# OpenSpaceAI/Nesie

Hardware: AMD Instinct MI355X
Metric: ScanNet scenes/sec (fwd+bwd, 40k pts, bs=8) (higher is better)
Workload: dtype f32; 1 GPU; Nesie-VoteNet supervised pretrain step (nesie-votenet-scannet-pretrain-10%): fwd+bwd+AdamW, 40000 pts/scene, fp32, random-init weights; scenes_per_gpu=8, global_batch=8, parallelism=single, world_size=1, hip_graph=True, deterministic_backward=True, index_chain_pipelined=True, forward_cu_budget=232, forward_cu_budget_from_the_head_on=248, grad_allreduce_bytes=10561936, resident_input_scenes=0

## Files before the change

nesie_amd/csrc/interpolate.hip:

```cpp
#include "common.h"
#include <math.h>

namespace nesie {

constexpr int NN_BLOCK = 256;
constexpr int NN_TILE = 1024;

template <int FORM>
__global__ __launch_bounds__(NN_BLOCK) void three_nn_kernel(
    int n, int m, const float *__restrict__ unknown, const float *__restrict__ known,
    float *__restrict__ dist2, int *__restrict__ idx) {
  __shared__ float4 kk[NN_TILE];
  const int bi = blockIdx.y;
  const int q = blockIdx.x * NN_BLOCK + threadIdx.x;
  const bool live = q < n;
  unknown += (size_t)bi * n * 3;
  known += (size_t)bi * m * 3;
  const int qq = live ? q : n - 1;
  const float ux = unknown[qq * 3 + 0], uy = unknown[qq * 3 + 1], uz = unknown[qq * 3 + 2];
  float b1 = INFINITY, b2 = INFINITY, b3 = INFINITY;
  int i1 = 0, i2 = 0, i3 = 0;
  for (int t0 = 0; t0 < m; t0 += NN_TILE) {
    const int tn = m - t0 < NN_TILE ? m - t0 : NN_TILE;
    __syncthreads();
    for (int i = threadIdx.x; i < tn; i += NN_BLOCK)
      kk[i] = make_float4(known[(t0 + i) * 3 + 0], known[(t0 + i) * 3 + 1],
                          known[(t0 + i) * 3 + 2], 0.f);
    __syncthreads();
#pragma unroll 4
    for (int i = 0; i < tn; ++i) {
      const float4 kp = kk[i];
      const float d = sqdist_form<FORM>(ux - kp.x, uy - kp.y, uz - kp.z);
      if (d < b3) {
        const int k = t0 + i;
        if (d < b1) {
          b3 = b2; i3 = i2; b2 = b1; i2 = i1; b1 = d; i1 = k;
        } else if (d < b2) {
          b3 = b2; i3 = i2; b2 = d; i2 = k;
        } else {
          b3 = d; i3 = k;
        }
      }
    }
  }
  if (live) {
    float *od = dist2 + ((size_t)bi * n + q) * 3;
    int *oi = idx + ((size_t)bi * n + q) * 3;
    od[0] = b1; od[1] = b2; od[2] = b3;
    oi[0] = i1; oi[1] = i2; oi[2] = i3;
  }
}

template <int FORM>
__global__ __launch_bounds__(NN_BLOCK) void grid_taps_kernel(
    int kprop, int gp, int m, const float *__restrict__ centre, const float *__restrict__ size,
    const float *__restrict__ heading, const float *__restrict__ mult,
    const float *__restrict__ plane, const float *__restrict__ known, int *__restrict__ idx,
    float *__restrict__ weight, float *__restrict__ rel) {
  __shared__ float4 kk[NN_TILE];
  const int bi = blockIdx.y;
  const int n = kprop * gp;
  const int q = blockIdx.x * NN_BLOCK + threadIdx.x;
  const bool live = q < n;
  const int qq = live ? q : n - 1;
  const int k = qq / gp, g = qq - k * gp;
  const float *c3 = centre + ((size_t)bi * kprop + k) * 3;
  const float *s3 = size + ((size_t)bi * kprop + k) * 3;
  const float cx = c3[0], cy = c3[1], cz = c3[2];
  float l[3];
#pragma unroll
  for (int d = 0; d < 3; ++d) {
    const float f = __fmul_rn(mult[g * 3 + d], s3[d]) / 2.f;
    l[d] = __fadd_rn(f, __fmul_rn(f, plane[g * 3 + d]));
  }
  const float h = heading[(size_t)bi * kprop + k];
  const float ch = cosf(h), sh = sinf(h);
  const float ux = __fadd_rn(__fadd_rn(__fmul_rn(l[0], ch), __fmul_rn(l[1], sh)), cx);
  const float uy = __fadd_rn(__fadd_rn(__fmul_rn(l[0], -sh), __fmul_rn(l[1], ch)), cy);
  const float uz = __fadd_rn(l[2], cz);
  known += (size_t)bi * m * 3;
  float b1 = INFINITY, b2 = INFINITY, b3 = INFINITY;
  int i1 = 0, i2 = 0, i3 = 0;
  for (int t0 = 0; t0 < m; t0 += NN_TILE) {
    const int tn = m - t0 < NN_TILE ? m - t0 : NN_TILE;
    __syncthreads();
    for (int i = threadIdx.x; i < tn; i += NN_BLOCK)
      kk[i] = make_float4(known[(t0 + i) * 3 + 0], known[(t0 + i) * 3 + 1],
                          known[(t0 + i) * 3 + 2], 0.f);
    __syncthreads();
#pragma unroll 4
    for (int i = 0; i < tn; ++i) {
      const float4 kp = kk[i];
      const float d = sqdist_form<FORM>(ux - kp.x, uy - kp.y, uz - kp.z);
      if (d < b3) {
        const int kidx = t0 + i;
        if (d < b1) {
          b3 = b2; i3 = i2; b2 = b1; i2 = i1; b1 = d; i1 = kidx;
        } else if (d < b2) {
          b3 = b2; i3 = i2; b2 = d; i2 = kidx;
        } else {
          b3 = d; i3 = kidx;
        }
      }
    }
  }
  if (live) {
    const size_t o = ((size_t)bi * n + q) * 3;
    const float w1 = 1.f / __fadd_rn(sqrtf(b1), 1e-8f), w2 = 1.f / __fadd_rn(sqrtf(b2), 1e-8f),
                w3 = 1.f / __fadd_rn(sqrtf(b3), 1e-8f);
    const float ws = __fadd_rn(__fadd_rn(w1, w2), w3);
    idx[o] = i1; idx[o + 1] = i2; idx[o + 2] = i3;
    weight[o] = w1 / ws; weight[o + 1] = w2 / ws; weight[o + 2] = w3 / ws;
    rel[o] = ux - cx; rel[o + 1] = uy - cy; rel[o + 2] = uz - cz;
  }
}

constexpr int TI_BLOCK = 256;
constexpr int TI_CH = 8;

__global__ __launch_bounds__(TI_BLOCK) void three_interpolate_kernel(
    int c, int m, int n, const float *__restrict__ points, const int *__restrict__ idx,
    const float *__restrict__ weight, float *__restrict__ out) {
  const int p = blockIdx.x * TI_BLOCK + threadIdx.x;
  const int c0 = blockIdx.y * TI_CH;
  const int bi = blockIdx.z;
  if (p >= n) return;
  const int *ix = idx + ((size_t)bi * n + p) * 3;
  const float *w = weight + ((size_t)bi * n + p) * 3;
  int j0 = ix[0], j1 = ix[1], j2 = ix[2];
  j0 = j0 < 0 ? 0 : (j0 >= m ? m - 1 : j0);
  j1 = j1 < 0 ? 0 : (j1 >= m ? m - 1 : j1);
  j2 = j2 < 0 ? 0 : (j2 >= m ? m - 1 : j2);
  const float w0 = w[0], w1 = w[1], w2 = w[2];
  const int cend = c - c0 < TI_CH ? c - c0 : TI_CH;
#pragma unroll
  for (int i = 0; i < TI_CH; ++i) {
    if (i < cend) {
      const float *src = points + ((size_t)bi * c + c0 + i) * m;
      float r = __fadd_rn(__fadd_rn(__fmul_rn(w0, src[j0]), __fmul_rn(w1, src[j1])),
                          __fmul_rn(w2, src[j2]));
      out[((size_t)bi * c + c0 + i) * n + p] = r;
    }
  }
}

constexpr int TS_Q = 64;

__global__ __launch_bounds__(256) void blend_fwd_kernel(
    int c, int m, int n, int segs, int seg_len, int c_total, int c_offset, int pitch,
    int seg_off, const float *__restrict__ table, const int *__restrict__ idx,
    const float *__restrict__ weight, const float *__restrict__ rel,
    const float *__restrict__ wx, float *__restrict__ out, float *__restrict__ stat_partial,
    int nt, int nb) {
  __shared__ float tile[64][TS_Q + 1];
  __shared__ float red[4][64][2];
  __shared__ int sj[TS_Q][3];
  __shared__ float sw[TS_Q][3];
  __shared__ float sr[TS_Q][3];
  const int bi = blockIdx.x % nb;
  const int q0 = (blockIdx.x / nb) * TS_Q;
  const int per_seg = n / segs;
  const int sg = q0 / per_seg, r0 = q0 - sg * per_seg;
  const int lane = threadIdx.x & 63, wv = threadIdx.x >> 6;
  if (threadIdx.x < TS_Q) {
    const int r = r0 + threadIdx.x;
    const int k = r / seg_len, g = r - k * seg_len;
    const size_t p = (size_t)bi * n + (size_t)(k * segs + sg) * seg_len + g;
#pragma unroll
    for (int t = 0; t < 3; ++t) {
      int j = idx[p * 3 + t];
      sj[threadIdx.x][t] = j < 0 ? 0 : (j >= m ? m - 1 : j);
      sw[threadIdx.x][t] = weight[p * 3 + t];
      sr[threadIdx.x][t] = rel ? rel[p * 3 + t] : 0.f;
    }
  }
  __syncthreads();
  const float *feat = table + (size_t)bi * m * pitch + (size_t)sg * seg_off;
  float *dst = out + (((size_t)bi * segs + sg) * c_total + c_offset) * per_seg + r0;
  for (int c0 = 0; c0 < c; c0 += 64) {
    float x0 = 0.f, x1 = 0.f, x2 = 0.f;
    if (wx) {
      const float *wr = wx + ((size_t)sg * c + c0 + lane) * 3;
      x0 = wr[0]; x1 = wr[1]; x2 = wr[2];
    }
    float a_s = 0.f, a_q = 0.f;
#pragma unroll 4
    for (int i = 0; i < 16; ++i) {
      const int qi = wv * 16 + i;
      const float *f = feat + c0 + lane;
      const float a0 = f[(size_t)sj[qi][0] * pitch], a1 = f[(size_t)sj[qi][1] * pitch],
                  a2 = f[(size_t)sj[qi][2] * pitch];
      float v = __fadd_rn(__fadd_rn(__fmul_rn(sw[qi][0], a0), __fmul_rn(sw[qi][1], a1)),
                          __fmul_rn(sw[qi][2], a2));
      if (wx)
        v = __fadd_rn(__fadd_rn(__fadd_rn(v, __fmul_rn(x0, sr[qi][0])), __fmul_rn(x1, sr[qi][1])),
                      __fmul_rn(x2, sr[qi][2]));
      tile[lane][qi] = v;
      a_s += v; a_q += v * v;
    }
    if (stat_partial) { red[wv][lane][0] = a_s; red[wv][lane][1] = a_q; }
    __syncthreads();
#pragma unroll
    for (int i = 0; i < 4; ++i) {
      const int ch = wv * 16 + i * 4 + (lane >> 4), q4 = (lane & 15) * 4;
      const float4 v = make_float4(tile[ch][q4], tile[ch][q4 + 1], tile[ch][q4 + 2], tile[ch][q4 + 3]);
      float *o = dst + (size_t)(c0 + ch) * per_seg + q4;
      if (nt) st4<true>(o, v); else st4<false>(o, v);
    }
    if (stat_partial && wv == 0) {
      const float ss = (red[0][lane][0] + red[1][lane][0]) + (red[2][lane][0] + red[3][lane][0]);
      const float qq = (red[0][lane][1] + red[1][lane][1]) + (red[2][lane][1] + red[3][lane][1]);
      const int nslice = nb * (per_seg / TS_Q);
      const int slice = bi * (per_seg / TS_Q) + r0 / TS_Q;
      float *pd = stat_partial + ((size_t)(sg * c + c0 + lane) * nslice + slice) * 2;
      pd[0] = ss; pd[1] = qq;
    }
    __syncthreads();
  }
}

__global__ __launch_bounds__(TI_BLOCK) void blend_fwd_generic_kernel(
    int c, int m, int n, int segs, int seg_len, int c_total, int c_offset, int pitch,
    int seg_off, const float *__restrict__ table, const int *__restrict__ idx,
    const float *__restrict__ weight, const float *__restrict__ rel,
    const float *__restrict__ wx, float *__restrict__ out) {
  const int q = blockIdx.x * TI_BLOCK + threadIdx.x;
  const int c0 = blockIdx.y * TI_CH;
  const int bi = blockIdx.z;
  if (q >= n) return;
  const int per_seg = n / segs;
  const int sg = q / per_seg, r = q - sg * per_seg;
  const int k = r / seg_len, g = r - k * seg_len;
  const size_t p = (size_t)bi * n + (size_t)(k * segs + sg) * seg_len + g;
  int j0 = idx[p * 3], j1 = idx[p * 3 + 1], j2 = idx[p * 3 + 2];
  j0 = j0 < 0 ? 0 : (j0 >= m ? m - 1 : j0);
  j1 = j1 < 0 ? 0 : (j1 >= m ? m - 1 : j1);
  j2 = j2 < 0 ? 0 : (j2 >= m ? m - 1 : j2);
  const float w0 = weight[p * 3], w1 = weight[p * 3 + 1], w2 = weight[p * 3 + 2];
  const float rx = rel ? rel[p * 3] : 0.f, ry = rel ? rel[p * 3 + 1] : 0.f,
              rz = rel ? rel[p * 3 + 2] : 0.f;
  const int cend = c - c0 < TI_CH ? c - c0 : TI_CH;
  const float *feat = table + (size_t)bi * m * pitch + (size_t)sg * seg_off + c0;
  float *dst = out + (((size_t)bi * segs + sg) * c_total + c_offset + c0) * per_seg + r;
#pragma unroll
  for (int i = 0; i < TI_CH; ++i) {
    if (i < cend) {
      float v = __fadd_rn(
          __fadd_rn(__fmul_rn(w0, feat[(size_t)j0 * pitch + i]), __fmul_rn(w1, feat[(size_t)j1 * pitch + i])),
          __fmul_rn(w2, feat[(size_t)j2 * pitch + i]));
      if (wx) {
        const float *wr = wx + ((size_t)sg * c + c0 + i) * 3;
        v = __fadd_rn(__fadd_rn(__fadd_rn(v, __fmul_rn(wr[0], rx)), __fmul_rn(wr[1], ry)),
                      __fmul_rn(wr[2], rz));
      }
      dst[(size_t)i * per_seg] = v;
    }
  }
}

constexpr int BL_RUN = 512;

__device__ __forceinline__ unsigned bitonic_sort64(unsigned v, int lane) {
#pragma unroll
  for (int k = 2; k <= 64; k <<= 1) {
#pragma unroll
    for (int j = k >> 1; j >= 1; j >>= 1) {
      const unsigned o = (unsigned)__shfl_xor((int)v, j, 64);
      const bool up = (lane & k) == 0;
      const bool lower = (lane & j) == 0;
      v = (up == lower) ? (v < o ? v : o) : (v > o ? v : o);
    }
  }
  return v;
}

constexpr int BL_SLOTS = 48;

template <int CPT, bool BNB, bool STAGED>
__global__ __launch_bounds__(256, 2) void blend_bwd_rows_kernel(
    int m, int n, int segs, int seg_len, int pitch, int seg_off,
    const float *__restrict__ dy , const int *__restrict__ idx,
    const float *__restrict__ weight, const float *__restrict__ rel,
    float *__restrict__ d_table, float *__restrict__ d_wx_part, int nb, int nruns,
    const float *__restrict__ bnz, const float *__restrict__ bnb,
    float *__restrict__ stage, int *__restrict__ slot_seed) {
  constexpr int C = CPT * 64;
  __shared__ float tile[C * (TS_Q + 1)];
  __shared__ int sj[TS_Q][3];
  __shared__ float sw[TS_Q][3];
  __shared__ float sr[TS_Q][3];
  const int bi = blockIdx.x % nb, run_i = (blockIdx.x / nb) % nruns, sg = blockIdx.x / (nb * nruns);
  const int per_seg = n / segs;
  const int run0 = run_i * BL_RUN;
  const int lane = threadIdx.x & 63, wv = threadIdx.x >> 6;
  const float *src = dy + ((size_t)bi * segs + sg) * C * per_seg;
  const float *zsrc = BNB ? bnz + ((size_t)bi * segs + sg) * C * per_seg : nullptr;
  const int wvu = __builtin_amdgcn_readfirstlane(wv);
  float *dt = d_table + (size_t)bi * m * pitch + (size_t)sg * seg_off + lane;
  float dx[CPT][3];
#pragma unroll
  for (int e = 0; e < CPT; ++e) dx[e][0] = dx[e][1] = dx[e][2] = 0.f;
  const int run_end = run0 + BL_RUN < per_seg ? run0 + BL_RUN : per_seg;
  constexpr int NR = C / 4;
  float traw[NR], zraw[BNB ? NR : 1];
  int pj[3];
  float pw[3], pr[3];
  auto prefetch = [&](int r0) {
    if (threadIdx.x < TS_Q) {
      const int r = r0 + threadIdx.x;
      const int k = r / seg_len, g = r - k * seg_len;
      const size_t p = (size_t)bi * n + (size_t)(k * segs + sg) * seg_len + g;
#pragma unroll
      for (int t = 0; t < 3; ++t) {
        pj[t] = idx[p * 3 + t];
        pw[t] = weight[p * 3 + t];
        pr[t] = rel ? rel[p * 3 + t] : 0.f;
      }
    }
    const unsigned voff = (unsigned)(((size_t)wv * per_seg + lane) * 4);
#pragma unroll
    for (int i = 0; i < NR; ++i) {
      const float *sb_ = src + (size_t)(i * 4) * per_seg + r0;
      traw[i] = *(const float *)((const char *)sb_ + voff);
    }
  };
  auto load_z = [&](int r0) {
    const unsigned voff = (unsigned)(((size_t)wv * per_seg + lane) * 4);
#pragma unroll
    for (int i = 0; i < NR; ++i) {
      const float *zb_ = zsrc + (size_t)(i * 4) * per_seg + r0;
      zraw[i] = *(const float *)((const char *)zb_ + voff);
    }
  };
  auto lds_barrier = [&]() {
    asm volatile("s_waitcnt lgkmcnt(0)" ::: "memory");
    __builtin_amdgcn_s_barrier();
  };
  if (run0 < run_end) prefetch(run0);
  for (int r0 = run0; r0 < run_end; r0 += TS_Q) {
    if (BNB) load_z(r0);
    lds_barrier();
    if (threadIdx.x < TS_Q) {
#pragma unroll
      for (int t = 0; t < 3; ++t) {
        const int j = pj[t];
        sj[threadIdx.x][t] = j < 0 ? 0 : (j >= m ? m - 1 : j);
        sw[threadIdx.x][t] = pw[t];
        sr[threadIdx.x][t] = pr[t];
      }
    }
#pragma unroll
    for (int i = 0; i < NR; ++i) {
      float v = traw[i];
      if (BNB) {
        const float *cf = bnb + ((size_t)sg * C + i * 4 + wvu) * 8;
        const float zz = zraw[i];
        const float gg = __builtin_fmaf(zz, cf[0], cf[1]) > 0.f ? v : 0.f;
        v = __builtin_fmaf(cf[2], gg, __builtin_fmaf(cf[3] - zz, cf[4], cf[5]));
      }
      tile[(i * 4 + wv) * (TS_Q + 1) + lane] = v;
    }
    lds_barrier();
    const int rn = r0 + TS_Q < run_end ? r0 + TS_Q : r0;
    prefetch(rn);
    const int q0 = wv * 16;
    if (d_wx_part) {
#pragma unroll 4
      for (int u = 0; u < 16; ++u) {
        const float r0x = sr[q0 + u][0], r1x = sr[q0 + u][1], r2x = sr[q0 + u][2];
#pragma unroll
        for (int e = 0; e < CPT; ++e) {
          const float v = tile[(e * 64 + lane) * (TS_Q + 1) + q0 + u];
          dx[e][0] += v * r0x; dx[e][1] += v * r1x; dx[e][2] += v * r2x;
        }
      }
    }
    unsigned key = 0xFFFFFFFFu;
    if (lane < 48) key = ((unsigned)sj[q0 + lane / 3][lane % 3] << 6) | (unsigned)lane;
    key = bitonic_sort64(key, lane);
    int cur = -1;
    float acc[CPT];
#pragma unroll
    for (int e = 0; e < CPT; ++e) acc[e] = 0.f;
    const size_t gslot = STAGED ? ((size_t)((size_t)bi * segs + sg) * (per_seg / 16) + (r0 + q0) / 16) * BL_SLOTS : 0;
    int rank = 0;
    if (STAGED) {
      const int sd = lane < 48 ? (int)(key >> 6) : -1;
      const int sp = __shfl_up(sd, 1, 64);
      const bool first = lane < 48 && (lane == 0 || sd != sp);
      const unsigned long long fm = __ballot(first);
      const int nvalid = __popcll(fm);
      if (first) slot_seed[gslot + __popcll(fm & ((1ull << lane) - 1ull))] = sd;
      if (lane >= nvalid && lane < BL_SLOTS) slot_seed[gslot + lane] = -1;
    }
    auto emit = [&]() {
      if (STAGED) {
        float *row = stage + (gslot + rank) * C + lane;
#pragma unroll
        for (int e = 0; e < CPT; ++e) row[e * 64] = acc[e];
        ++rank;
      } else {
#pragma unroll
        for (int e = 0; e < CPT; ++e) atomicAdd(dt + (size_t)cur * pitch + e * 64, acc[e]);
      }
    };
#pragma unroll 1
    for (int i0 = 0; i0 < 48; i0 += 8) {
      int seeds[8];
      float x[8][CPT];
#pragma unroll
      for (int i = 0; i < 8; ++i) {
        const unsigned u = (unsigned)__builtin_amdgcn_readlane((int)key, i0 + i);
        const int tap = (int)(u & 63u);
        const int q = q0 + tap / 3, t = tap % 3;
        seeds[i] = (int)(u >> 6);
        const float w = sw[q][t];
#pragma unroll
        for (int e = 0; e < CPT; ++e) x[i][e] = tile[(e * 64 + lane) * (TS_Q + 1) + q] * w;
      }
#pragma unroll
      for (int i = 0; i < 8; ++i) {
        if (seeds[i] != cur) {
          if (cur >= 0) emit();
          cur = seeds[i];
#pragma unroll
          for (int e = 0; e < CPT; ++e) acc[e] = 0.f;
        }
#pragma unroll
        for (int e = 0; e < CPT; ++e) acc[e] += x[i][e];
      }
    }
    emit();
  }
  if (d_wx_part) {
    __syncthreads();
    float *red = tile;
#pragma unroll
    for (int e = 0; e < CPT; ++e)
#pragma unroll
      for (int d = 0; d < 3; ++d) red[(wv * C + e * 64 + lane) * 3 + d] = dx[e][d];
    __syncthreads();
    float *dst = d_wx_part + ((((size_t)bi * nruns + run_i) * segs + sg) * C) * 3;
    for (int i = threadIdx.x; i < C * 3; i += 256)
      dst[i] = (red[i] + red[C * 3 + i]) + (red[2 * C * 3 + i] + red[3 * C * 3 + i]);
  }
}

constexpr int SI_GROUPS = 128;
constexpr int SI_BLOCK = 1024, SI_WAVES = SI_BLOCK / 64;
constexpr int SI_MAX_BINS = 2048;

__global__ __launch_bounds__(SI_BLOCK) void blend_slot_index_kernel(
    int m, int groups_per_face, int nchunk, const int *__restrict__ slot_seed,
    int *__restrict__ order, int *__restrict__ offs) {
  extern __shared__ int si_lds[];
  int *cnt = si_lds, *scratch = si_lds + SI_WAVES * m;
  const int face = blockIdx.x / nchunk, chunk = blockIdx.x % nchunk;
  const int tid = threadIdx.x, lane = tid & 63;
  const int wave = __builtin_amdgcn_readfirstlane(tid >> 6);
  const int g0 = chunk * SI_GROUPS;
  const int g1 = g0 + SI_GROUPS < groups_per_face ? g0 + SI_GROUPS : groups_per_face;
  const int *ss = slot_seed + (size_t)face * groups_per_face * BL_SLOTS;
  for (int j = tid; j < SI_WAVES * m; j += SI_BLOCK) cnt[j] = 0;
  __syncthreads();
  constexpr int GPW = SI_GROUPS / SI_WAVES;
  int *mine = cnt + wave * m;
  int sv[GPW];
#pragma unroll
  for (int u = 0; u < GPW; ++u) {
    const int g = g0 + wave * GPW + u;
    int v = -1;
    if (g < g1 && lane < BL_SLOTS) v = ss[(size_t)g * BL_SLOTS + lane];
    sv[u] = (v >= 0 && v < m) ? v : -1;
  }
#pragma unroll
  for (int u = 0; u < GPW; ++u)
    if (sv[u] >= 0) atomicAdd(&mine[sv[u]], 1);
  __syncthreads();
  const int bper = (m + SI_BLOCK - 1) / SI_BLOCK;
  const int b0 = tid * bper, b1 = b0 + bper < m ? b0 + bper : m;
  int sum = 0;
  for (int sbin = b0; sbin < b1; ++sbin)
    for (int w = 0; w < SI_WAVES; ++w) sum += cnt[w * m + sbin];
  scratch[tid] = sum;
  __syncthreads();
  for (int d = 1; d < SI_BLOCK; d <<= 1) {
    const int v = tid >= d ? scratch[tid - d] : 0;
    __syncthreads();
    scratch[tid] += v;
    __syncthreads();
  }
  int *of = offs + ((size_t)face * nchunk + chunk) * (m + 1);
  int run = scratch[tid] - sum;
  for (int sbin = b0; sbin < b1; ++sbin) {
    of[sbin] = run;
    for (int w = 0; w < SI_WAVES; ++w) {
      const int c = cnt[w * m + sbin];
      cnt[w * m + sbin] = run;
      run += c;
    }
  }
  if (tid == SI_BLOCK - 1) of[m] = scratch[SI_BLOCK - 1];
  __syncthreads();
  int *ord = order + ((size_t)face * nchunk + chunk) * (SI_GROUPS * BL_SLOTS);
#pragma unroll
  for (int u = 0; u < GPW; ++u) {
    if (sv[u] >= 0) {
      const int pos = atomicAdd(&mine[sv[u]], 1);
      ord[pos] = (g0 + wave * GPW + u) * BL_SLOTS + lane;
    }
  }
}

template <int CPT>
__global__ __launch_bounds__(256) void blend_bwd_gather_kernel(
    int m, int segs, int pitch, int seg_off, int slots_per_face, int nchunk,
    const float *__restrict__ stage, const int *__restrict__ order, const int *__restrict__ offs,
    float *__restrict__ d_table, int nb) {
  constexpr int C = CPT * 64;
  struct Row {
    float v[CPT];
    __device__ __forceinline__ void load(const float *p) {
      if constexpr (CPT == 4) { const float4 t = *(const float4 *)p; v[0] = t.x; v[1] = t.y; v[2] = t.z; v[3] = t.w; }
      else if constexpr (CPT == 2) { const float2 t = *(const float2 *)p; v[0] = t.x; v[1] = t.y; }
      else {
#pragma unroll
        for (int e = 0; e < CPT; ++e) v[e] = p[e];
      }
    }
    __device__ __forceinline__ void store(float *p) const {
      if constexpr (CPT == 4) *(float4 *)p = make_float4(v[0], v[1], v[2], v[3]);
      else if constexpr (CPT == 2) *(float2 *)p = make_float2(v[0], v[1]);
      else {
#pragma unroll
        for (int e = 0; e < CPT; ++e) p[e] = v[e];
      }
    }
  };
  const int lane = threadIdx.x & 63;
  const long long w = (long long)blockIdx.x * 4 + (threadIdx.x >> 6);
  if (w >= (long long)nb * segs * m) return;
  const int seed = (int)(w % m), face = (int)(w / m);
  const int bi = face / segs, sg = face % segs;
  int lo = 0, hi = 0;
  if (lane < nchunk) {
    const int *of = offs + ((size_t)face * nchunk + lane) * (m + 1) + seed;
    lo = of[0]; hi = of[1];
  }
  const float *base = stage + (size_t)face * slots_per_face * C + lane * CPT;
  Row acc;
#pragma unroll
  for (int e = 0; e < CPT; ++e) acc.v[e] = 0.f;
  for (int ch = 0; ch < nchunk; ++ch) {
    const int l = __builtin_amdgcn_readlane(lo, ch), h = __builtin_amdgcn_readlane(hi, ch);
    const int *ob = order + ((size_t)face * nchunk + ch) * (SI_GROUPS * BL_SLOTS);
    for (int j0 = l; j0 < h; j0 += 64) {
      const int cntj = h - j0 < 64 ? h - j0 : 64;
      const int myslot = lane < cntj ? ob[j0 + lane] : 0;
      int u = 0;
      for (; u + 3 < cntj; u += 4) {
        Row v[4];
#pragma unroll
        for (int k = 0; k < 4; ++k) v[k].load(base + (size_t)__builtin_amdgcn_readlane(myslot, u + k) * C);
#pragma unroll
        for (int k = 0; k < 4; ++k)
#pragma unroll
          for (int e = 0; e < CPT; ++e) acc.v[e] += v[k].v[e];
      }
      for (; u < cntj; ++u) {
        Row v;
        v.load(base + (size_t)__builtin_amdgcn_readlane(myslot, u) * C);
#pragma unroll
        for (int e = 0; e < CPT; ++e) acc.v[e] += v.v[e];
      }
    }
  }
  acc.store(d_table + ((size_t)bi * m + seed) * pitch + (size_t)sg * seg_off + lane * CPT);
}

__global__ __launch_bounds__(TI_BLOCK) void three_interpolate_grad_kernel(
    int c, int n, int m, const float *__restrict__ grad_out, const int *__restrict__ idx,
    const float *__restrict__ weight, float *__restrict__ grad_points) {
  const int p = blockIdx.x * TI_BLOCK + threadIdx.x;
  const int c0 = blockIdx.y * TI_CH;
  const int bi = blockIdx.z;
  if (p >= n) return;
  const int *ix = idx + ((size_t)bi * n + p) * 3;
  const float *w = weight + ((size_t)bi * n + p) * 3;
  int j0 = ix[0], j1 = ix[1], j2 = ix[2];
  j0 = j0 < 0 ? 0 : (j0 >= m ? m - 1 : j0);
  j1 = j1 < 0 ? 0 : (j1 >= m ? m - 1 : j1);
  j2 = j2 < 0 ? 0 : (j2 >= m ? m - 1 : j2);
  const float w0 = w[0], w1 = w[1], w2 = w[2];
  const int cend = c - c0 < TI_CH ? c - c0 : TI_CH;
#pragma unroll
  for (int i = 0; i < TI_CH; ++i) {
    if (i < cend) {
      const float g = grad_out[((size_t)bi * c + c0 + i) * n + p];
      float *dst = grad_points + ((size_t)bi * c + c0 + i) * m;
      atomicAdd(dst + j0, __fmul_rn(g, w0));
      atomicAdd(dst + j1, __fmul_rn(g, w1));
      atomicAdd(dst + j2, __fmul_rn(g, w2));
    }
  }
}

}

using namespace nesie;

extern "C" int nesie_three_nn_wrapper(int b, int n, int m, const float *unknown,
                                      const float *known, float *dist2, int *idx,
                                      void *stream) {
  const char *W = "three_nn_wrapper";
  NESIE_REQUIRE(b >= 0 && n >= 0 && m >= 0, W);
  if (b == 0 || n == 0) return NESIE_OK;
  NESIE_REQUIRE(unknown && dist2 && idx && (m == 0 || known), W);
  NESIE_REQUIRE(b <= 65535 && (long long)n * 3 < (1ll << 31) && (long long)m * 3 < (1ll << 31), W);
#define NN(FORM)                                                                          \
  hipLaunchKernelGGL(three_nn_kernel<FORM>, dim3(cdiv(n, NN_BLOCK), b), dim3(NN_BLOCK), 0, \
                     (hipStream_t)stream, n, m, unknown, known, dist2, idx)
  if (distance_form() == 1) NN(1);
  else if (distance_form() == 2) NN(2);
  else NN(0);
#undef NN
  return check_launch(W);
}

extern "C" int nesie_grid_taps(int b, int kprop, int gp, int m, const float *centre,
                               const float *size, const float *heading, const float *mult,
                               const float *plane, const float *known, int *idx, float *weight,
                               float *rel, void *stream) {
  const char *W = "grid_taps";
  NESIE_REQUIRE(b >= 0 && kprop >= 0 && gp >= 0 && m >= 0, W);
  if (b == 0 || kprop == 0 || gp == 0) return NESIE_OK;
  NESIE_REQUIRE(m >= 3 && centre && size && heading && mult && plane && known, W);
  NESIE_REQUIRE(idx && weight && rel && b <= 65535 && (long long)kprop * gp * 3 < (1ll << 31), W);
#define GT(FORM)                                                                                \
  hipLaunchKernelGGL(grid_taps_kernel<FORM>, dim3(cdiv((long long)kprop * gp, NN_BLOCK), b),     \
                     dim3(NN_BLOCK), 0, (hipStream_t)stream, kprop, gp, m, centre, size, heading, \
                     mult, plane, known, idx, weight, rel)
  if (distance_form() == 1) GT(1);
  else if (distance_form() == 2) GT(2);
  else GT(0);
#undef GT
  return check_launch(W);
}

extern "C" int nesie_three_interpolate_wrapper(int b, int c, int m, int n,
                                               const float *points, const int *idx,
                                               const float *weight, float *out,
                                               void *stream) {
  const char *W = "three_interpolate_wrapper";
  NESIE_REQUIRE(b >= 0 && c >= 0 && m >= 0 && n >= 0, W);
  if (b == 0 || c == 0 || n == 0) return NESIE_OK;
  NESIE_REQUIRE(m >= 1 && points && idx && weight && out, W);
  NESIE_REQUIRE(b <= 65535 && cdiv(c, TI_CH) <= 65535, W);
  hipLaunchKernelGGL(three_interpolate_kernel, dim3(cdiv(n, TI_BLOCK), cdiv(c, TI_CH), b),
                     dim3(TI_BLOCK), 0, (hipStream_t)stream, c, m, n, points, idx, weight,
                     out);
  return check_launch(W);
}

static int blend_check(const char *W, int b, int c, int m, int n, int segs, int seg_len,
                       int pitch, int seg_off) {
  NESIE_REQUIRE(b >= 0 && c >= 0 && m >= 0 && n >= 0 && segs >= 1 && seg_len >= 1, W);
  NESIE_REQUIRE(n % (segs * seg_len) == 0 && seg_off >= 0, W);
  NESIE_REQUIRE(pitch >= (long long)(segs - 1) * seg_off + c, W);
  NESIE_REQUIRE(b <= 65535 && cdiv(c, TI_CH) <= 65535, W);
  return NESIE_OK;
}

extern "C" int nesie_blend_conv_forward(int b, int c, int m, int n, const float *table,
                                        int pitch, int seg_off, const int *idx,
                                        const float *weight, const float *rel, const float *wx,
                                        float *out, int segs, int seg_len, int c_total,
                                        int c_offset, float *stat_partial, void *stream) {
  const char *W = "blend_conv_forward";
  int st = blend_check(W, b, c, m, n, segs, seg_len, pitch, seg_off);
  if (st) return st;
  NESIE_REQUIRE(c_offset >= 0 && c_offset + c <= c_total && (wx == nullptr) == (rel == nullptr), W);
  if (b == 0 || c == 0 || n == 0) return NESIE_OK;
  NESIE_REQUIRE(m >= 1 && table && idx && weight && out, W);
  if (stat_partial && !(c % 64 == 0 && (n / segs) % TS_Q == 0)) {
    set_error("%s: stat_partial needs c %% 64 == 0 and %d-multiple faces", W, TS_Q);
    return NESIE_ERR_UNSUPPORTED;
  }
  if (c % 64 == 0 && (n / segs) % TS_Q == 0)
    hipLaunchKernelGGL(blend_fwd_kernel, dim3((n / TS_Q) * b), dim3(256), 0, (hipStream_t)stream, c,
                       m, n, segs, seg_len, c_total, c_offset, pitch, seg_off, table, idx, weight,
                       rel, wx, out, stat_partial, 0, b);
  else
    hipLaunchKernelGGL(blend_fwd_generic_kernel, dim3(cdiv(n, TI_BLOCK), cdiv(c, TI_CH), b),
                       dim3(TI_BLOCK), 0, (hipStream_t)stream, c, m, n, segs, seg_len, c_total,
                       c_offset, pitch, seg_off, table, idx, weight, rel, wx, out);
  return check_launch(W);
}

extern "C" int nesie_blend_conv_runs(int n, int segs) {
  return segs >= 1 && n >= 0 ? cdiv(n / segs, BL_RUN) : 0;
}

static size_t blend_stage_slots(int b, int n, int segs) { return (size_t)b * (n / 16) * BL_SLOTS; }
static int blend_index_chunks(int n, int segs) { return cdiv(n / segs / 16, SI_GROUPS); }

extern "C" size_t nesie_blend_conv_backward_workspace_bytes(int b, int c, int n, int segs) {
  if (b <= 0 || c <= 0 || n <= 0 || segs <= 0) return 0;
  const size_t slots = blend_stage_slots(b, n, segs);
  const size_t order_ints = (size_t)b * segs * blend_index_chunks(n, segs) * SI_GROUPS * BL_SLOTS;
  const size_t offs_ints = (size_t)b * segs * blend_index_chunks(n, segs) * SI_MAX_BINS;
  return slots * c * sizeof(float) + (slots + order_ints + offs_ints) * sizeof(int);
}

static int blend_conv_backward_impl(const char *W, int b, int c, int m, int n, const float *dy,
                                    int pitch, int seg_off, const int *idx, const float *weight,
                                    const float *rel, float *d_table, float *d_wx, int segs,
                                    int seg_len, const float *bnz, const float *bnb, void *stream,
                                    void *workspace = nullptr, size_t workspace_bytes = 0) {
  int st = blend_check(W, b, c, m, n, segs, seg_len, pitch, seg_off);
  if (st) return st;
  if (b == 0 || c == 0 || n == 0) return NESIE_OK;
  NESIE_REQUIRE(m >= 1 && dy && idx && weight && d_table && segs <= 65535, W);
  NESIE_REQUIRE((d_wx == nullptr) || rel, W);
  const int per_seg = n / segs;
  if (c % 64 != 0 || c > 256 || per_seg % TS_Q != 0) {
    set_error("%s: c %d (needs 64, 128, 192 or 256) / %d queries per face (needs a multiple "
              "of %d)", W, c, per_seg, TS_Q);
    return NESIE_ERR_UNSUPPORTED;
  }
  const int nruns = cdiv(per_seg, BL_RUN);
  NESIE_REQUIRE((long long)nruns * b * segs < (1ll << 31), W);
  const dim3 grid((unsigned)(nruns * b * segs));
  hipStream_t s = (hipStream_t)stream;
  if (workspace) {
    const size_t slots = blend_stage_slots(b, n, segs);
    NESIE_REQUIRE(workspace_bytes >= nesie_blend_conv_backward_workspace_bytes(b, c, n, segs), W);
    NESIE_REQUIRE(((uintptr_t)workspace & 15) == 0 && m + 1 <= SI_MAX_BINS, W);
    NESIE_REQUIRE(pitch % 4 == 0 && seg_off % 4 == 0 && ((uintptr_t)d_table & 15) == 0, W);
    const int groups_per_face = per_seg / 16, slots_per_face = groups_per_face * BL_SLOTS;
    const int nchunk = blend_index_chunks(n, segs);
    NESIE_REQUIRE(nchunk <= 64 && (long long)b * segs * nchunk < (1ll << 31) &&
                  (long long)b * segs * m < (1ll << 33), W);
    float *stage = (float *)workspace;
    int *slot_seed = (int *)(stage + slots * c), *order = slot_seed + slots,
        *offs = order + (size_t)b * segs * nchunk * SI_GROUPS * BL_SLOTS;
#define LS(N)                                                                                      \
  do {                                                                                             \
    if (bnb)                                                                                       \
      hipLaunchKernelGGL((blend_bwd_rows_kernel<N, true, true>), grid, dim3(256), 0, s,            \
                         m, n, segs, seg_len, pitch, seg_off, dy, idx, weight, rel, d_table, d_wx, \
                         b, nruns, bnz, bnb, stage, slot_seed);                                    \
    else                                                                                           \
      hipLaunchKernelGGL((blend_bwd_rows_kernel<N, false, true>), grid, dim3(256), 0, s,           \
                         m, n, segs, seg_len, pitch, seg_off, dy, idx, weight, rel, d_table, d_wx, \
                         b, nruns, bnz, bnb, stage, slot_seed);                                    \
  } while (0)
    if (c == 64) LS(1); else if (c == 128) LS(2); else if (c == 192) LS(3); else LS(4);
#undef LS
    {
      const size_t lds = ((size_t)SI_WAVES * m + SI_BLOCK) * sizeof(int);
      static bool attr = false;
      if (!attr) {
        (void)hipFuncSetAttribute((const void *)blend_slot_index_kernel, hipFuncAttributeMaxDynamicSharedMemorySize,
                                  (int)(((size_t)SI_WAVES * SI_MAX_BINS + SI_BLOCK) * sizeof(int)));
        attr = true;
      }
      hipLaunchKernelGGL(blend_slot_index_kernel, dim3((unsigned)(b * segs * nchunk)), dim3(SI_BLOCK), lds, s,
                         m, groups_per_face, nchunk, slot_seed, order, offs);
    }
    const long long waves = (long long)b * segs * m;
#define LG(N) hipLaunchKernelGGL((blend_bwd_gather_kernel<N>), dim3((unsigned)cdiv(waves, 4)), dim3(256), 0, s, \
                                 m, segs, pitch, seg_off, slots_per_face, nchunk, stage, order, offs, d_table, b)
    if (c == 64) LG(1); else if (c == 128) LG(2); else if (c == 192) LG(3); else LG(4);
#undef LG
    return check_launch(W);
  }
#define L(N)                                                                                       \
  do {                                                                                             \
    if (bnb)                                                                                       \
      hipLaunchKernelGGL((blend_bwd_rows_kernel<N, true, false>), grid, dim3(256), 0, s,           \
                         m, n, segs, seg_len, pitch, seg_off, dy, idx, weight, rel, d_table, d_wx, \
                         b, nruns, bnz, bnb, (float *)nullptr, (int *)nullptr);                    \
    else                                                                                           \
      hipLaunchKernelGGL((blend_bwd_rows_kernel<N, false, false>), grid, dim3(256), 0, s,          \
                         m, n, segs, seg_len, pitch, seg_off, dy, idx, weight, rel, d_table, d_wx, \
                         b, nruns, bnz, bnb, (float *)nullptr, (int *)nullptr);                    \
  } while (0)
  if (c == 64) L(1); else if (c == 128) L(2); else if (c == 192) L(3); else L(4);
#undef L
  return check_launch(W);
}

extern "C" int nesie_blend_conv_backward_staged(int b, int c, int m, int n, const float *dy, const float *z,
                                                const float *bnb, int pitch, int seg_off, const int *idx,
                                                const float *weight, const float *rel, float *d_table,
                                                float *d_wx, int segs, int seg_len, void *workspace,
                                                size_t workspace_bytes, void *stream) {
  const char *W = "blend_conv_backward_staged";
  NESIE_REQUIRE(workspace && (z == nullptr) == (bnb == nullptr), W);
  return blend_conv_backward_impl(W, b, c, m, n, dy, pitch, seg_off, idx, weight, rel, d_table, d_wx, segs,
                                  seg_len, z, bnb, stream, workspace, workspace_bytes);
}

extern "C" int nesie_blend_conv_backward(int b, int c, int m, int n, const float *dy,
                                         int pitch, int seg_off, const int *idx,
                                         const float *weight, const float *rel,
                                         float *d_table, float *d_wx, int segs, int seg_len,
                                         void *stream) {
  return blend_conv_backward_impl("blend_conv_backward", b, c, m, n, dy, pitch, seg_off, idx, weight, rel,
                                  d_table, d_wx, segs, seg_len, nullptr, nullptr, stream);
}

extern "C" int nesie_blend_conv_backward_bn(int b, int c, int m, int n, const float *da, const float *z,
                                            const float *bnb, int pitch, int seg_off, const int *idx,
                                            const float *weight, const float *rel, float *d_table,
                                            float *d_wx, int segs, int seg_len, void *stream) {
  const char *W = "blend_conv_backward_bn";
  NESIE_REQUIRE(b == 0 || c == 0 || n == 0 || (z && bnb), W);
  return blend_conv_backward_impl(W, b, c, m, n, da, pitch, seg_off, idx, weight, rel, d_table, d_wx, segs,
                                  seg_len, z, bnb, stream);
}

extern "C" int nesie_three_interpolate_grad_wrapper(int b, int c, int n, int m,
                                                    const float *grad_out,
                                                    const int *idx, const float *weight,
                                                    float *grad_points, void *stream) {
  const char *W = "three_interpolate_grad_wrapper";
  NESIE_REQUIRE(b >= 0 && c >= 0 && m >= 0 && n >= 0, W);
  if (b == 0 || c == 0 || n == 0) return NESIE_OK;
  NESIE_REQUIRE(m >= 1 && grad_out && idx && weight && grad_points, W);
  NESIE_REQUIRE(b <= 65535 && cdiv(c, TI_CH) <= 65535, W);
  hipLaunchKernelGGL(three_interpolate_grad_kernel,
                     dim3(cdiv(n, TI_BLOCK), cdiv(c, TI_CH), b), dim3(TI_BLOCK), 0,
                     (hipStream_t)stream, c, n, m, grad_out, idx, weight, grad_points);
  return check_launch(W);
}
```

Measured before the change: 680.0 scenes/s.

## Restructure blend forward kernel: per-thread channel vectors, grid over channel chunks, readlane indices

The blend forward kernel no longer loops over 64-channel slabs in one block. Channels are now split across a second grid dimension, and each thread handles CPT contiguous channels with vector loads. Neighbour indices, weights and rel offsets are now kept in registers and broadcast with readlane instead of shared memory, and the arithmetic uses packed float2 operations. The WX and STAT variants are compile-time template parameters, and the output always uses non-temporal stores. These changes aim to raise parallelism and memory-level parallelism in the gather. The costs are more dynamic LDS per block, up to two launches, and a reordered channel mapping whose rounding must still match the old results.

After: 687.8 scenes/s (median of 6 runs). 1.01x the previous value.

```diff
diff --git a/nesie_amd/csrc/interpolate.hip b/nesie_amd/csrc/interpolate.hip
--- a/nesie_amd/csrc/interpolate.hip
+++ b/nesie_amd/csrc/interpolate.hip
@@ -145,77 +145,129 @@
 }
 
 constexpr int TS_Q = 64;
-
+constexpr int BF_LD = TS_Q + 1;
+typedef float bf_f2 __attribute__((ext_vector_type(2)));
+constexpr int BF_NQ = 8;
+
+template <int CPT, bool WX, bool STAT>
 __global__ __launch_bounds__(256) void blend_fwd_kernel(
-    int c, int m, int n, int segs, int seg_len, int c_total, int c_offset, int pitch,
+    int c, int cb, int m, int n, int segs, int seg_len, int c_total, int c_offset, int pitch,
     int seg_off, const float *__restrict__ table, const int *__restrict__ idx,
     const float *__restrict__ weight, const float *__restrict__ rel,
     const float *__restrict__ wx, float *__restrict__ out, float *__restrict__ stat_partial,
-    int nt, int nb) {
-  __shared__ float tile[64][TS_Q + 1];
-  __shared__ float red[4][64][2];
-  __shared__ int sj[TS_Q][3];
-  __shared__ float sw[TS_Q][3];
-  __shared__ float sr[TS_Q][3];
+    int nb) {
+#pragma clang fp contract(off)
+  constexpr int CW = CPT * 64;
+  extern __shared__ float bf_lds[];
+  float *tile = bf_lds;
+  float *red = bf_lds + CW * BF_LD;
   const int bi = blockIdx.x % nb;
   const int q0 = (blockIdx.x / nb) * TS_Q;
+  const int c0 = cb + blockIdx.y * CW;
   const int per_seg = n / segs;
   const int sg = q0 / per_seg, r0 = q0 - sg * per_seg;
   const int lane = threadIdx.x & 63, wv = threadIdx.x >> 6;
-  if (threadIdx.x < TS_Q) {
-    const int r = r0 + threadIdx.x;
+  int pj[3];
+  float pw[3], pr[3];
+  {
+    const int r = r0 + wv * 16 + (lane & 15);
     const int k = r / seg_len, g = r - k * seg_len;
     const size_t p = (size_t)bi * n + (size_t)(k * segs + sg) * seg_len + g;
 #pragma unroll
     for (int t = 0; t < 3; ++t) {
-      int j = idx[p * 3 + t];
-      sj[threadIdx.x][t] = j < 0 ? 0 : (j >= m ? m - 1 : j);
-      sw[threadIdx.x][t] = weight[p * 3 + t];
-      sr[threadIdx.x][t] = rel ? rel[p * 3 + t] : 0.f;
+      const int j = idx[p * 3 + t];
+      pj[t] = j < 0 ? 0 : (j >= m ? m - 1 : j);
+      pw[t] = weight[p * 3 + t];
+      pr[t] = WX ? rel[p * 3 + t] : 0.f;
+    }
+  }
+  const float *feat = table + (size_t)bi * m * pitch + (size_t)sg * seg_off + c0;
+  const unsigned voff = (unsigned)(lane * CPT * 4);
+  float x[CPT][3] = {};
+  if (WX) {
+    __builtin_memcpy(&x[0][0], wx + ((size_t)sg * c + c0 + lane * CPT) * 3, sizeof(x));
+  }
+  constexpr int CP2 = CPT / 2;
+  bf_f2 s2[CP2 ? CP2 : 1], q2[CP2 ? CP2 : 1];
+  float s1 = 0.f, q1 = 0.f;
+#pragma unroll
+  for (int e = 0; e < CP2; ++e) s2[e] = q2[e] = bf_f2{0.f, 0.f};
+#pragma unroll
+  for (int i0 = 0; i0 < 16; i0 += BF_NQ) {
+    float a[BF_NQ][3][CPT];
+#pragma unroll
+    for (int i = 0; i < BF_NQ; ++i)
+#pragma unroll
+      for (int t = 0; t < 3; ++t) {
+        const int j = __builtin_amdgcn_readlane(pj[t], i0 + i);
+        const float *row = feat + (size_t)j * pitch;
+        __builtin_memcpy(a[i][t], (const char *)row + voff, CPT * 4);
+      }
+    __builtin_amdgcn_sched_barrier(0);
+#pragma unroll
+    for (int i = 0; i < BF_NQ; ++i) {
+      const int qi = wv * 16 + i0 + i;
+      float sw[3], sr[3];
+#pragma unroll
+      for (int t = 0; t < 3; ++t) {
+        sw[t] = __int_as_float(__builtin_amdgcn_readlane(__float_as_int(pw[t]), i0 + i));
+        sr[t] = __int_as_float(__builtin_amdgcn_readlane(__float_as_int(pr[t]), i0 + i));
+      }
+      auto blend = [&](auto a0, auto a1, auto a2, auto x0, auto x1, auto x2) {
+        auto v = (a0 * sw[0] + a1 * sw[1]) + a2 * sw[2];
+        if (WX) v = ((v + x0 * sr[0]) + x1 * sr[1]) + x2 * sr[2];
+        return v;
+      };
+#pragma unroll
+      for (int h = 0; h < CP2; ++h) {
+        const int e = 2 * h;
+        const bf_f2 v = blend(bf_f2{a[i][0][e], a[i][0][e + 1]}, bf_f2{a[i][1][e], a[i][1][e + 1]},
+                              bf_f2{a[i][2][e], a[i][2][e + 1]}, bf_f2{x[e][0], x[e + 1][0]},
+                              bf_f2{x[e][1], x[e + 1][1]}, bf_f2{x[e][2], x[e + 1][2]});
+        tile[(e * 64 + lane) * BF_LD + qi] = v.x;
+        tile[((e + 1) * 64 + lane) * BF_LD + qi] = v.y;
+        if (STAT) {
+          s2[h] = s2[h] + v;
+          q2[h] = q2[h] + v * v;
+        }
+      }
+      if (CPT & 1) {
+        constexpr int e = CPT - 1;
+        const float v = blend(a[i][0][e], a[i][1][e], a[i][2][e], x[e][0], x[e][1], x[e][2]);
+        tile[(e * 64 + lane) * BF_LD + qi] = v;
+        if (STAT) {
+          s1 = s1 + v;
+          q1 = q1 + v * v;
+        }
+      }
+    }
+  }
+  if (STAT) {
+#pragma unroll
+    for (int e = 0; e < CPT; ++e) {
+      const bool odd = (CPT & 1) && e == CPT - 1;
+      red[((wv * CW) + e * 64 + lane) * 2] = odd ? s1 : s2[e / 2][e & 1];
+      red[((wv * CW) + e * 64 + lane) * 2 + 1] = odd ? q1 : q2[e / 2][e & 1];
     }
   }
   __syncthreads();
-  const float *feat = table + (size_t)bi * m * pitch + (size_t)sg * seg_off;
-  float *dst = out + (((size_t)bi * segs + sg) * c_total + c_offset) * per_seg + r0;
-  for (int c0 = 0; c0 < c; c0 += 64) {
-    float x0 = 0.f, x1 = 0.f, x2 = 0.f;
-    if (wx) {
-      const float *wr = wx + ((size_t)sg * c + c0 + lane) * 3;
-      x0 = wr[0]; x1 = wr[1]; x2 = wr[2];
-    }
-    float a_s = 0.f, a_q = 0.f;
-#pragma unroll 4
-    for (int i = 0; i < 16; ++i) {
-      const int qi = wv * 16 + i;
-      const float *f = feat + c0 + lane;
-      const float a0 = f[(size_t)sj[qi][0] * pitch], a1 = f[(size_t)sj[qi][1] * pitch],
-                  a2 = f[(size_t)sj[qi][2] * pitch];
-      float v = __fadd_rn(__fadd_rn(__fmul_rn(sw[qi][0], a0), __fmul_rn(sw[qi][1], a1)),
-                          __fmul_rn(sw[qi][2], a2));
-      if (wx)
-        v = __fadd_rn(__fadd_rn(__fadd_rn(v, __fmul_rn(x0, sr[qi][0])), __fmul_rn(x1, sr[qi][1])),
-                      __fmul_rn(x2, sr[qi][2]));
-      tile[lane][qi] = v;
-      a_s += v; a_q += v * v;
-    }
-    if (stat_partial) { red[wv][lane][0] = a_s; red[wv][lane][1] = a_q; }
-    __syncthreads();
-#pragma unroll
-    for (int i = 0; i < 4; ++i) {
-      const int ch = wv * 16 + i * 4 + (lane >> 4), q4 = (lane & 15) * 4;
-      const float4 v = make_float4(tile[ch][q4], tile[ch][q4 + 1], tile[ch][q4 + 2], tile[ch][q4 + 3]);
-      float *o = dst + (size_t)(c0 + ch) * per_seg + q4;
-      if (nt) st4<true>(o, v); else st4<false>(o, v);
-    }
-    if (stat_partial && wv == 0) {
-      const float ss = (red[0][lane][0] + red[1][lane][0]) + (red[2][lane][0] + red[3][lane][0]);
-      const float qq = (red[0][lane][1] + red[1][lane][1]) + (red[2][lane][1] + red[3][lane][1]);
-      const int nslice = nb * (per_seg / TS_Q);
-      const int slice = bi * (per_seg / TS_Q) + r0 / TS_Q;
-      float *pd = stat_partial + ((size_t)(sg * c + c0 + lane) * nslice + slice) * 2;
-      pd[0] = ss; pd[1] = qq;
-    }
-    __syncthreads();
+  float *dst = out + (((size_t)bi * segs + sg) * c_total + c_offset + c0) * per_seg + r0;
+#pragma unroll
+  for (int i = 0; i < 4 * CPT; ++i) {
+    const int row = wv * (16 * CPT) + i * 4 + (lane >> 4), q4 = (lane & 15) * 4;
+    const int ch = (row & 63) * CPT + (row >> 6);
+    const float *tr = tile + row * BF_LD + q4;
+    st4<true>(dst + (size_t)ch * per_seg + q4, make_float4(tr[0], tr[1], tr[2], tr[3]));
+  }
+  if (STAT && threadIdx.x < CW) {
+    const int row = threadIdx.x, ch = (row & 63) * CPT + (row >> 6);
+    const float *rd = red + row * 2;
+    const float ss = (rd[0] + rd[CW * 2]) + (rd[2 * CW * 2] + rd[3 * CW * 2]);
+    const float qq = (rd[1] + rd[CW * 2 + 1]) + (rd[2 * CW * 2 + 1] + rd[3 * CW * 2 + 1]);
+    const int nslice = nb * (per_seg / TS_Q);
+    const int slice = bi * (per_seg / TS_Q) + r0 / TS_Q;
+    float *pd = stat_partial + ((size_t)(sg * c + c0 + ch) * nslice + slice) * 2;
+    pd[0] = ss; pd[1] = qq;
   }
 }
 
@@ -671,6 +723,32 @@
   return NESIE_OK;
 }
 
+template <int CPT>
+static void blend_fwd_launch(int chunks, int cb, int b, int c, int m, int n, int segs, int seg_len,
+                             int c_total, int c_offset, int pitch, int seg_off, const float *table,
+                             const int *idx, const float *weight, const float *rel, const float *wx,
+                             float *out, float *stat_partial, hipStream_t s) {
+  if (chunks <= 0) return;
+  constexpr int CW = CPT * 64;
+  const size_t lds = (size_t)CW * (BF_LD + 4 * 2) * sizeof(float);
+  const dim3 grid((unsigned)((n / TS_Q) * b), (unsigned)chunks);
+#define BF(WXF, STF)                                                                              \
+  do {                                                                                            \
+    static bool attr = false;                                                                     \
+    if (!attr) {                                                                                  \
+      (void)hipFuncSetAttribute((const void *)blend_fwd_kernel<CPT, WXF, STF>,                    \
+                                hipFuncAttributeMaxDynamicSharedMemorySize, (int)lds);            \
+      attr = true;                                                                                \
+    }                                                                                             \
+    hipLaunchKernelGGL((blend_fwd_kernel<CPT, WXF, STF>), grid, dim3(256), lds, s, c, cb, m, n,   \
+                       segs, seg_len, c_total, c_offset, pitch, seg_off, table, idx, weight, rel, \
+                       wx, out, stat_partial, b);                                                 \
+  } while (0)
+  if (wx) { if (stat_partial) BF(true, true); else BF(true, false); }
+  else { if (stat_partial) BF(false, true); else BF(false, false); }
+#undef BF
+}
+
 extern "C" int nesie_blend_conv_forward(int b, int c, int m, int n, const float *table,
                                         int pitch, int seg_off, const int *idx,
                                         const float *weight, const float *rel, const float *wx,
@@ -686,11 +764,16 @@
     set_error("%s: stat_partial needs c %% 64 == 0 and %d-multiple faces", W, TS_Q);
     return NESIE_ERR_UNSUPPORTED;
   }
-  if (c % 64 == 0 && (n / segs) % TS_Q == 0)
-    hipLaunchKernelGGL(blend_fwd_kernel, dim3((n / TS_Q) * b), dim3(256), 0, (hipStream_t)stream, c,
-                       m, n, segs, seg_len, c_total, c_offset, pitch, seg_off, table, idx, weight,
-                       rel, wx, out, stat_partial, 0, b);
-  else
+  if (c % 64 == 0 && (n / segs) % TS_Q == 0) {
+    NESIE_REQUIRE((long long)(n / TS_Q) * b < (1ll << 31) && ((uintptr_t)out & 15) == 0, W);
+    blend_fwd_launch<4>(c / 256, 0, b, c, m, n, segs, seg_len, c_total, c_offset, pitch, seg_off, table,
+                        idx, weight, rel, wx, out, stat_partial, (hipStream_t)stream);
+    const int cb = c / 256 * 256, left = (c - cb) / 64;
+#define REST(N) blend_fwd_launch<N>(1, cb, b, c, m, n, segs, seg_len, c_total, c_offset, pitch, seg_off, table, \
+                                    idx, weight, rel, wx, out, stat_partial, (hipStream_t)stream)
+    if (left == 1) REST(1); else if (left == 2) REST(2); else if (left == 3) REST(3);
+#undef REST
+  } else
     hipLaunchKernelGGL(blend_fwd_generic_kernel, dim3(cdiv(n, TI_BLOCK), cdiv(c, TI_CH), b),
                        dim3(TI_BLOCK), 0, (hipStream_t)stream, c, m, n, segs, seg_len, c_total,
                        c_offset, pitch, seg_off, table, idx, weight, rel, wx, out);
```
